# junhuihe2000/FLGP

Hardware: AMD Instinct MI355X
Metric: points/sec through k-NN->Laplacian->trunc-SVD->heat-cov, n=1e6 d=16 K=200 (higher is better)
Workload: dtype f64

## Files before the change

flgp_amd/_lib.py:

```python
from __future__ import annotations

import ctypes
import os

_HERE = os.path.dirname(os.path.abspath(__file__))
LIB_PATH = os.path.join(_HERE, "libflgp_hip.so")

c_int, c_double, c_long, c_void_p, c_char_p, c_size_t = (
    ctypes.c_int, ctypes.c_double, ctypes.c_long, ctypes.c_void_p, ctypes.c_char_p, ctypes.c_size_t)

P = c_void_p
_SIGNATURES = {
    "flgp_last_error": (c_char_p, []),
    "flgp_version": (c_char_p, []),
    "flgp_device_count": (c_int, []),
    "flgp_dev_pool_release": (c_size_t, []),
    "flgp_release_pinned": (None, []),
    "flgp_set_device": (c_int, [c_int]),
    "flgp_parse_gl": (c_int, [c_char_p]),
    "flgp_set_tuning": (c_int, [c_char_p, c_int]),
    "flgp_prof_enable": (None, [c_int]),
    "flgp_prof_reset": (None, []),
    "flgp_prof_query": (c_int, [c_char_p, P, P, P]),
    "flgp_prof_names": (c_int, [P, c_int]),
# ... 115 lines not shown
    "flgp_dev_gram_pack": (c_int, [P, P, P, c_int, c_int, P]),
    "flgp_dev_sym_pack": (c_int, [P, P, c_int, c_int, P]),
    "flgp_dev_sym_unpack": (c_int, [P, P, c_int, P, c_int]),
    "flgp_dev_eig_workspace": (c_size_t, [c_int, c_int]),
    "flgp_dev_eig_topk": (c_int, [P, P, c_int, c_int, c_int, c_double, P, P, c_int, P, c_size_t, P]),
    "flgp_dev_eig_plan": (c_int, [c_int, c_int, P]),
    "flgp_dev_bsg_workspace": (c_size_t, [c_int, c_int]),
    "flgp_dev_bsg_set_trace": (None, [P]),
    "flgp_dev_jac_set_trace": (None, [P]),
    "flgp_dev_bsg_apply": (c_int, [P, P, c_int, c_int, P, c_int, c_double, c_double, P, P, P, c_size_t, P]),
    "flgp_dev_u_recover_workspace": (c_size_t, [c_int, c_int]),
    "flgp_dev_u_recover_route": (c_int, [c_int, c_int, c_int, c_int, c_int]),
    "flgp_dev_spectrum_usable": (c_int, [P, P, c_int]),
    "flgp_dev_spectrum_usable_route": (c_int, [P, P, c_int, c_int]),
    "flgp_dev_u_recover": (c_int, [P, P, P, c_int, c_int, P, c_int, c_int, P, c_int, c_double, c_int, P, c_int, P, P]),
    "flgp_dev_hk": (c_int, [P, P, c_int, c_double, P, c_int, P, c_int, c_int, P, c_int, P, c_int, c_int,
                            P, c_int, P]),
    "flgp_dev_cholesky": (c_int, [P, P, c_int, c_int, P]),
    "flgp_dev_chol_solve": (c_int, [P, P, c_int, P, c_int, c_int, P]),
    "flgp_dev_tri_inverse_workspace": (c_size_t, [c_int]),
    "flgp_dev_tri_inverse": (c_int, [P, P, c_int, P, P, c_size_t, P]),
    "flgp_dev_gemm": (c_int, [P, c_int, c_int, c_int, c_double, P, c_long, c_long, P, c_long, c_long,
                              c_double, P, c_long, c_long, P, c_long, c_long, P, c_size_t]),
    "flgp_dev_rotate": (c_int, [P, c_int, c_int, c_double, P, P, P, c_double, P, P, P]),
    "flgp_dev_gram_small": (c_int, [P, c_int, c_int, P, P, P, P, c_size_t]),
    "flgp_dev_gemm_pair": (c_int, [P, c_int, c_int, c_int, c_double, P, P, c_long, c_long, P, P, c_long, c_long, P, P, c_long, c_long]),
    "flgp_dev_gemm_ex": (c_int, [P, c_int, c_int, c_int, c_double, P, c_long, c_long, P, c_long, c_long,
                                 c_double, P, c_long, c_long, P, c_long, c_long, P, c_size_t, c_double,
                                 P, c_int, c_int, P, P, P, P, P, P, P, ctypes.POINTER(c_int)]),
    "flgp_dev_gram_small_fused": (c_int, [P, c_int, c_int, P, P, P, P, c_size_t, c_int, P, P, P, P]),
# ... 61 lines not shown
```

flgp_amd/csrc/capi.hip:

```cpp
#include "common.h"
#include <chrono>
#include <memory>
#include <cstring>
#include <cmath>
#include <string>
#include <thread>
#include <vector>

using namespace flgp;

extern "C" int flgp_dev_spectrum_usable_route(void *stream, const double *d_eig, int K, int full_decomposition) {
  hipStream_t st = (hipStream_t)stream;
  FLGP_REQUIRE(d_eig && K >= 1, "spectrum_usable: bad arguments");
  std::vector<double> hv((size_t)K);
  FLGP_HIP(hipMemcpyAsync(hv.data(), d_eig, sizeof(double) * (size_t)K, hipMemcpyDeviceToHost, st));
  FLGP_HIP(hipStreamSynchronize(st));
  const double top = hv[0], low = hv[K - 1];
  if (!(top > 0.0) || !std::isfinite(top)) { set_error("spectrum: the similarity matrix is zero or not finite"); return FLGP_ERR_INVALID; }
  const double floor_rel = full_decomposition ? std::pow(10.0, -(double)tuning("spectrum_floor_exp_full", 13))
                                              : std::pow(10.0, -(double)tuning("spectrum_floor_exp", 10));
  if (!(low > floor_rel * top)) {
    set_error("spectrum: sigma_%d^2 = %.3e is below %.0e sigma_1^2 (= %.3e), what the %s resolves: K = %d reaches into the "
              "(numerical) null space of the similarity matrix, whose left vectors the Gram route cannot recover -- choose a "
              "smaller K", K, low, floor_rel, top, full_decomposition ? "full decomposition" : "block eigensolver", K);
// ... 206 lines not shown
  return laplacian(S, st, gl, sizes);
}

int csr_out(Sim &S, hipStream_t st, int *csr_p, int *csr_j, double *csr_x) {
  FLGP_TRY(d2h(csr_j, S.ell_idx.p, sizeof(int) * (size_t)S.n * S.r, st));
  FLGP_TRY(d2h(csr_x, S.ell_val.p, sizeof(double) * (size_t)S.n * S.r, st));
  FLGP_HIP(hipStreamSynchronize(st));
  if (csr_p)
    for (long i = 0; i <= S.n; ++i) csr_p[i] = (int)(i * S.r);
  return FLGP_OK;
}

struct Spectrum {
  DevBuf G, rec, eig, V, values, vectors, work, uwork;
  int K = 0;
};

int spectrum(Sim &S, hipStream_t st, int K, int root, Spectrum &P, int *info) {
  if (K < 0) K = S.s;
  FLGP_REQUIRE(K >= 1 && K <= S.s, "need 1 <= K <= s (K=%d, s=%d)", K, S.s);
  P.K = K;
  FLGP_TRY(build_csc_async(S, st));
  FLGP_TRY(colsum_of(S, st, S.ell_idx.as<int>(), S.ell_val.as<double>()));
  FLGP_TRY(flgp_comm_all_reduce_sum(S.comm, S.colsum.as<double>(), (size_t)S.s, st));
  FLGP_TRY(keep_colsum(S, st, S.keep_colsum_spectrum));
  FLGP_TRY(flgp_dev_col_scale(st, S.ell_idx.as<int>(), S.ell_val.as<double>(), S.n, S.r, S.colsum.as<double>(), nullptr, 1));
  FLGP_TRY(P.G.alloc(sizeof(double) * (size_t)S.s * S.s));
  FLGP_TRY(join_csc(S, st));
  if (flgp_dev_gram_uses_records(S.s, S.r)) {
    FLGP_TRY(P.rec.alloc(flgp_dev_gram_record_bytes(S.n, S.r)));
    FLGP_TRY(flgp_dev_gram_pack(st, S.ell_idx.as<int>(), S.ell_val.as<double>(), S.n, S.r, P.rec.as<double>()));
  }
  FLGP_TRY(flgp_dev_gram_ordered(st, S.ell_idx.as<int>(), S.ell_val.as<double>(), S.n, S.s, S.r, S.colptr.as<int>(),
// ... 5 lines not shown
    FLGP_TRY(flgp_dev_sym_pack(st, P.G.as<double>(), S.s, S.s, packed.as<double>()));
    FLGP_TRY(flgp_comm_all_reduce_sum(S.comm, packed.as<double>(), cnt, st));
    FLGP_TRY(flgp_dev_sym_unpack(st, packed.as<double>(), S.s, P.G.as<double>(), S.s));
    FLGP_HIP(hipStreamSynchronize(st));
  }
  const size_t wb = flgp_dev_eig_workspace(S.s, K);
  FLGP_TRY(P.work.alloc(wb));
  FLGP_TRY(P.eig.alloc(sizeof(double) * (size_t)K));
  FLGP_TRY(P.V.alloc(sizeof(double) * (size_t)S.s * K));
  int solve_info[4] = {0, 0, 0, 0};
  FLGP_TRY(flgp_dev_eig_topk(st, P.G.as<double>(), S.s, S.s, K, 0.0, P.eig.as<double>(), P.V.as<double>(), S.s,
                             P.work.p, wb, solve_info));
  if (info) for (int q = 0; q < 4; ++q) info[q] = solve_info[q];
  FLGP_TRY(flgp_dev_spectrum_usable_route(st, P.eig.as<double>(), K, solve_info[2]));
  if (!P.values.p) FLGP_TRY(P.values.alloc(sizeof(double) * (size_t)K));
  if (!P.vectors.p) FLGP_TRY(P.vectors.alloc(sizeof(double) * (size_t)S.n * K));
  FLGP_TRY(P.uwork.alloc(flgp_dev_u_recover_workspace(S.s, K)));
  return flgp_dev_u_recover(st, S.ell_idx.as<int>(), S.ell_val.as<double>(), S.n, S.r, P.V.as<double>(), S.s, S.s,
                            P.eig.as<double>(), K, std::sqrt((double)(S.n_global ? S.n_global : (long)S.n)), root,
                            P.vectors.as<double>(), S.n, P.values.as<double>(), P.uwork.as<double>());
}

int parse_kernel(const char *kernel, int *se) {
  if (kernel && !strcmp(kernel, "lae")) { *se = 0; return FLGP_OK; }
  if (kernel && !strcmp(kernel, "se")) { *se = 1; return FLGP_OK; }
  set_error("The kernel type is not supported!");
  return FLGP_ERR_UNSUPPORTED;
}

double now_s() { return std::chrono::duration<double>(std::chrono::steady_clock::now().time_since_epoch()).count(); }

struct HostSpectrum {
  Stream st;
  Sim S;
  Spectrum P;
// ... 632 lines not shown
  if (glc < 0) return glc;
  FLGP_REQUIRE(dX_loc && dU && dH_loc, "sharded covariance: null pointer");
  FLGP_REQUIRE(n_loc >= 1 && ldx >= n_loc && d >= 1 && s >= 1 && ldu >= s, "sharded covariance: bad shape n_loc=%d d=%d s=%d", n_loc, d, s);
  FLGP_REQUIRE(n_global >= n_loc && row_lo >= 0 && row_lo + n_loc <= n_global, "sharded covariance: rows [%ld, %ld) do not lie in [0, %ld)",
               row_lo, row_lo + n_loc, n_global);
  FLGP_REQUIRE(m >= 1 && (long)m <= n_global && ldh >= n_loc, "sharded covariance: need 1 <= m <= n and ldh >= n_loc");
  FLGP_REQUIRE(glc != FLGP_GL_CLUSTER_NORMALIZED || d_sizes, "gl=\"cluster-normalized\" needs the cluster sizes");
  FLGP_REQUIRE(!d_vectors_out || ldv >= n_loc, "sharded covariance: ldv < n_loc");
  if (K < 0) K = s;
  Sim S;
  S.n = n_loc; S.d = d; S.s = s; S.ldx = ldx; S.comm = comm; S.n_global = n_global; S.sizes = d_sizes;
  S.X.borrow(dX_loc);
  FLGP_TRY(anchor_panel(st, dU, s, ldu, d, S.Ut, S.uu));
  S.want_csc = true;
  FLGP_TRY(cross_similarity(S, st, r, se, glc, epsilon, d));
  Spectrum P;
  FLGP_TRY(spectrum(S, st, K, root, P, info));
  DevBuf V1, work;
  FLGP_TRY(V1.alloc(sizeof(double) * (size_t)m * K));
  FLGP_HIP(hipMemsetAsync(V1.p, 0, sizeof(double) * (size_t)m * K, st));
  if (row_lo < m) {
    const long cnt = std::min<long>(row_lo + n_loc, (long)m) - row_lo;
    FLGP_HIP(hipMemcpy2DAsync(V1.as<double>() + row_lo, sizeof(double) * (size_t)m, P.vectors.p, sizeof(double) * (size_t)n_loc,
                              sizeof(double) * (size_t)cnt, K, hipMemcpyDeviceToDevice, st));
  }
  FLGP_TRY(flgp_comm_all_reduce_sum(comm, V1.as<double>(), (size_t)m * K, st));
  FLGP_TRY(work.alloc(flgp_dev_hk_workspace(n_loc, m, K, 0)));
  FLGP_TRY(flgp_dev_hk(st, P.values.as<double>(), K, t, P.vectors.as<double>(), n_loc, nullptr, 0, n_loc, V1.as<double>(), m, nullptr, 0,
                       m, dH_loc, ldh, work.as<double>()));
  if (d_values_out) FLGP_HIP(hipMemcpyAsync(d_values_out, P.values.p, sizeof(double) * (size_t)K, hipMemcpyDeviceToDevice, st));
  if (d_vectors_out)
    FLGP_HIP(hipMemcpy2DAsync(d_vectors_out, sizeof(double) * (size_t)ldv, P.vectors.p, sizeof(double) * (size_t)n_loc,
                              sizeof(double) * (size_t)n_loc, K, hipMemcpyDeviceToDevice, st));
  FLGP_HIP(hipStreamSynchronize(st));
  return FLGP_OK;
}

extern "C" int flgp_heat_kernel_covariance_rank(const flgp_comm *comm, const double *X_rows, long ldx_host, int n_loc,
                                                long n_global, long row_lo, int m, int d, const double *U, int s, int ucols,
                                                int r, double t, int K, const char *kernel, const char *gl, int root,
                                                double epsilon, double *H_rows, long ldh_host, int *info) {
  const int world = comm ? comm->world : 1;
  Stream st;
  DevBuf dX, dUall, dHl;
// ... 212 lines not shown
```

flgp_amd/csrc/common.h:

```cpp
#pragma once
#include <hip/hip_runtime.h>
#include <cstdarg>
#include <cstdio>
#include <cstring>
#include <vector>
#include "../../include/flgp_hip.h"
#include "worker_pool.h"

namespace flgp {

void set_error(const char *fmt, ...);
int tuning(const char *key, int dflt);

struct DeviceFigures { int cus, lds_per_block; };
DeviceFigures device_figures();

int prof_begin(const char *name, hipStream_t st, double work);
void prof_end(int idx, hipStream_t st);
struct ProfScope {
  int idx; hipStream_t st;
  ProfScope(const char *name, hipStream_t s, double work) : idx(prof_begin(name, s, work)), st(s) {}
  ~ProfScope() { prof_end(idx, st); }
};

// ... 153 lines not shown
                 GemmFusedReduce *fused);
bool rot_applicable(int s, int b, const double *X, const double *X2, const double *WT, const double *out, const double *out2);
int rot_launch(hipStream_t st, int s, int b, double alpha, const double *X, const double *X2, const double *WT, double beta,
               const double *E, const double *E2, double *out, double *out2);
constexpr int GEMM_DIST_PARTS = 32;
struct GemmFusedReduce {
  int mode;
  double *dinv, *dist, *scratch;
  int *counter;
  bool done;
};

bool hk_panel_applicable(int n0, int n1, int K, long ldh);
bool hk_panel2_applicable(int n0, int n1, int K, long ldh);
size_t hk_panel_vw_elems(int n1, int K);
int hk_panel2_launch(hipStream_t st, const double *d_values, int K, double t, const double *V0, long ld0, int n0,
                     const double *dV1, int ld1, const int *d_idx1, int row0_1, int n1, double *dH, long ldh,
                     double *d_vw);
int hk_panel_launch(hipStream_t st, const double *d_values, int K, double t, const double *V0, long ld0, int n0,
                    const double *dV1, int ld1, const int *d_idx1, int row0_1, int n1, double *dH, long ldh,
                    double *d_vw);

int hk_ranges_to_host(hipStream_t st, const double *d_values, int K, double t, const double *d_vectors, int ldv,
                      int row0_0, int n0, int row0_1, int n1, double *H);
int d2h_cols_pipelined(hipStream_t st, const double *dM, long rows, int cols, double *H, long ldh, int rings_at_least);

int chol_solve(hipStream_t st, double *dA, int N, double *dB, int nrhs, int *d_flag);
int gpr_weights(hipStream_t st, const double *d_values, int K, double t, double *d_ls, double *d_l);
int gpr_q(hipStream_t st, const double *dVtV, const double *d_ls, int K, double c, double *dQ);
int gpr_scale(hipStream_t st, const double *dM, const double *d_a, const double *d_b, int rows, int cols, double *d_out);
// ... 174 lines not shown
```

flgp_amd/csrc/gemm.hip:

```cpp
#include "common.h"
#include <type_traits>

namespace flgp {

typedef double d4 __attribute__((ext_vector_type(4)));
typedef double d2 __attribute__((ext_vector_type(2)));

constexpr int GB = 128;
constexpr int GK = 16;
#ifndef GEMM_GLD_PAD
#define GEMM_GLD_PAD 17
#endif
constexpr int gld_of(int gbt) { return gbt + GEMM_GLD_PAD; }

struct GemmArgs {
  int M, N, Kd;
  const double *A; long a_is, a_ks;
  const double *B; long b_ks, b_js;
  double alpha, beta, gamma;
  const double *E; long e_is, e_js;
  const double *E2;
  double *C; long c_is, c_js;
  int shift_edges;
  int ksplit_len;
// ... 583 lines not shown
    FLGP_TRY(check_launch("splitk_reduce_kernel"));
  }
  return FLGP_OK;
}

__global__ void hk_scale_kernel(const double *__restrict__ values, int K, double t, const double *__restrict__ V1,
                                int ld1, const int *__restrict__ idx1, int row0, int n1, double *__restrict__ Vw) {
  const long e = (long)blockIdx.x * blockDim.x + threadIdx.x;
  if (e >= (long)n1 * K) return;
  const int b = (int)(e % n1), k = (int)(e / n1);
  const int row = idx1 ? idx1[b] : row0 + b;
  const double w = exp(-t * (1.0 - values[k]));
  Vw[e] = V1[(size_t)k * ld1 + row] * w;
}

__global__ void gather_rows_kernel(const double *__restrict__ V, int ld, const int *__restrict__ idx, int n0, int K,
                                   double *__restrict__ out, int ldo) {
  const long e = (long)blockIdx.x * blockDim.x + threadIdx.x;
  if (e >= (long)n0 * K) return;
  const int a = (int)(e % n0), k = (int)(e / n0);
  out[(size_t)k * ldo + a] = V[(size_t)k * ld + idx[a]];
}

}

using namespace flgp;

extern "C" int flgp_dev_gemm(void *stream, int M, int N, int Kd, double alpha, const double *A, long a_is,
                             long a_ks, const double *B, long b_ks, long b_js, double beta, const double *E,
                             long e_is, long e_js, double *C, long c_is, long c_js, double *d_work,
// ... 85 lines not shown
  double *Vw = d_work;
  const double *V0 = dV0 + row0_0;
  long v0_ld = ld0;
  if (d_idx0) {
    double *G0 = d_work + hk_panel_vw_elems(n1, K);
    hipLaunchKernelGGL(gather_rows_kernel, dim3(ceil_div((long)n0 * K, 256)), dim3(256), 0, st, dV0, ld0, d_idx0,
                       n0, K, G0, n0);
    FLGP_TRY(check_launch("gather_rows_kernel"));
    V0 = G0;
    v0_ld = n0;
  }
  if (hk_panel2_applicable(n0, n1, K, ldh))
    return hk_panel2_launch(st, d_values, K, t, V0, v0_ld, n0, dV1, ld1, d_idx1, row0_1, n1, dH, ldh, Vw);
  if (hk_panel_applicable(n0, n1, K, ldh))
    return hk_panel_launch(st, d_values, K, t, V0, v0_ld, n0, dV1, ld1, d_idx1, row0_1, n1, dH, ldh, Vw);
  hipLaunchKernelGGL(hk_scale_kernel, dim3(ceil_div((long)n1 * K, 256)), dim3(256), 0, st, d_values, K, t, dV1, ld1,
                     d_idx1, row0_1, n1, Vw);
  FLGP_TRY(check_launch("hk_scale_kernel"));
  return gemm_launch(st, n0, n1, K, 1.0, V0, 1, v0_ld, Vw, n1, 1, 0.0, nullptr, 0, 0, dH, 1, ldh, nullptr, 0, 0.0,
                     nullptr);
}
```

flgp_amd/csrc/sparse.hip:

```cpp
#include "common.h"

namespace flgp {

__global__ __launch_bounds__(256) void csc_hist_kernel(const int *__restrict__ ell_idx, long nnz, int s,
                                                       int chunk, int *__restrict__ hist) {
  extern __shared__ int lh[];
  for (int j = threadIdx.x; j < s; j += blockDim.x) lh[j] = 0;
  __syncthreads();
  const long e0 = (long)blockIdx.x * chunk;
  long e1 = e0 + chunk;
  if (e1 > nnz) e1 = nnz;
  for (long e = e0 + threadIdx.x; e < e1; e += blockDim.x) atomicAdd(&lh[ell_idx[e]], 1);
  __syncthreads();
  int *out = hist + (size_t)blockIdx.x * s;
  for (int j = threadIdx.x; j < s; j += blockDim.x) out[j] = lh[j];
}

__global__ void csc_colscan_kernel(int *__restrict__ hist, int nchunks, int s, int *__restrict__ tot) {
  const int j = blockIdx.x * blockDim.x + threadIdx.x;
  if (j >= s) return;
  int run = 0;
  constexpr int CB = 16;
  int c = 0;
  for (; c + CB <= nchunks; c += CB) {
// ... 480 lines not shown
  }
  __syncthreads();
  for (int e = tid; e < KT * ROWS; e += 256) {
    const int kq = e / ROWS, i = e % ROWS;
    if (k0 + kq < K && i0 + i < n) out[(size_t)(k0 + kq) * ldo + i0 + i] = tile[kq][i];
  }
}

#ifndef U_RECOVER_LDS_THREADS
#define U_RECOVER_LDS_THREADS 1024
#endif
#ifndef U_RECOVER_LDS_MIN_N
#define U_RECOVER_LDS_MIN_N 10000
#endif
constexpr int U_LDS_BYTES = 163840;

static int u_lds_width(int s) {
  const long w = s >= 1 ? (long)U_LDS_BYTES / (8L * s) : 0;
  return w > 4 ? 4 : (int)w;
}

template <int W>
__global__ __launch_bounds__(256) void transpose_v_slices_kernel(const double *__restrict__ V, int ldv, int s, int K,
                                                                 double *__restrict__ Vts) {
  const int j = blockIdx.x * 256 + threadIdx.x, sl = blockIdx.y;
  if (j >= s) return;
  double *o = Vts + ((size_t)sl * s + j) * W;
#pragma unroll
  for (int c = 0; c < W; ++c) {
    const int k = sl * W + c;
    o[c] = k < K ? V[(size_t)k * ldv + j] : 0.0;
  }
}

template <int W> __device__ __forceinline__ int u_lds_slot(int q) { return W == 4 ? q ^ (((q >> 5) & 1) << 1) : q; }

template <int W, int NP>
__global__ __launch_bounds__(U_RECOVER_LDS_THREADS) void u_recover_lds_kernel(const int *__restrict__ ell_idx,
                                                                              const double *__restrict__ val, int n, int r, int s,
                                                                              const double *__restrict__ Vts,
                                                                              const double *__restrict__ eig, int K, double scale,
                                                                              double *__restrict__ out, int ldo, int rows_per_range) {
  typedef double d2u __attribute__((ext_vector_type(2), aligned(8)));
  typedef int i2u __attribute__((ext_vector_type(2), aligned(4)));
  typedef double d2 __attribute__((ext_vector_type(2)));
  extern __shared__ __attribute__((aligned(16))) double u_slice[];
  const int tid = threadIdx.x, T = blockDim.x, sl = blockIdx.y;
  const double *src = Vts + (size_t)sl * s * W;
  for (int q = tid; q < s * W; q += T) u_slice[u_lds_slot<W>(q)] = src[q];
  double sg[W];
#pragma unroll
  for (int c = 0; c < W; ++c) {
    const int k = sl * W + c;
    const double e = k < K ? eig[k] : 0.0;
    sg[c] = __builtin_sqrt(e > 0.0 ? e : 0.0);
  }
  __syncthreads();
  const long i_lo = (long)blockIdx.x * rows_per_range;
  const long i_hi = (i_lo + rows_per_range < n) ? i_lo + rows_per_range : n;
  const long last_pair = (long)n * r - 2;
  constexpr int CE = 2 * NP;
  constexpr int GB = NP <= 4 ? CE : (W == 4 && NP == 6) ? 4 : NP;
  struct Chunk { double z0[NP], z1[NP]; int j0[NP], j1[NP]; };
  auto fetch = [&](long i, int ch) {
    Chunk c;
#pragma unroll
    for (int u = 0; u < NP; ++u) {
      const int a = CE * ch + 2 * u;
      long b = (i < i_hi && a < r) ? i * r + a : i_lo * r;
// ... 46 lines not shown
#pragma unroll
        for (int h = 0; h < 2; ++h)
          if (2 * u + h < left) {
            double z, v[W];
            gather(cur, u, h, moved, z, v);
#pragma unroll
            for (int c = 0; c < W; ++c) acc[c] += z * v[c];
          }
      }
    }
    if (ch == nch - 1) {
      if (i < i_hi) {
#pragma unroll
        for (int c = 0; c < W; ++c) {
          const int k = sl * W + c;
          if (k < K) out[(size_t)k * ldo + i] = sg[c] > 0.0 ? (acc[c] / sg[c]) * scale : 0.0;
        }
      }
#pragma unroll
      for (int c = 0; c < W; ++c) acc[c] = 0.0;
    }
  };
  const long nit = i_hi > i_lo ? (i_hi - i_lo + T - 1) / T : 0;
  const long steps = nit * nch;
  long ia = i_lo + tid; int cha = 0;
  auto next = [&](long &i, int &ch) { if (++ch == nch) { ch = 0; i += T; } };
  Chunk A = fetch(ia, cha), B;
  for (long t = 0; t < steps; t += 2) {
    long ib = ia; int chb = cha; next(ib, chb);
    B = fetch(ib, chb);
    apply(A, ia, cha);
    ia = ib; cha = chb; next(ia, cha);
    A = fetch(ia, cha);
    if (t + 1 < steps) apply(B, ib, chb);
  }
}

__global__ void values_out_kernel(const double *__restrict__ eig, int K, int root, double *__restrict__ values) {
  const int k = blockIdx.x * blockDim.x + threadIdx.x;
  if (k >= K) return;
  const double ev = eig[k] > 0.0 ? eig[k] : 0.0;
  values[k] = root ? __builtin_sqrt(ev) : ev;
}

struct CscPlan {
  int nchunks, chunk, nbits;
  size_t hist_bytes, tot_bytes;
};

static CscPlan csc_plan(long nnz, int s) {
  CscPlan p;
  long nc = (nnz + 2047) / 2048;
  if (nc > 2048) nc = 2048;
  if (nc < 1) nc = 1;
  long chunk = (nnz + nc - 1) / nc;
  chunk = (chunk + 63) / 64 * 64;
  if (chunk < 64) chunk = 64;
// ... 238 lines not shown
  int dev = 0;
  if (hipGetDevice(&dev) != hipSuccess || dev < 0 || dev >= 16) return 256;
  if (!cus[dev]) {
    int c = 0;
    cus[dev] = (hipDeviceGetAttribute(&c, hipDeviceAttributeMultiprocessorCount, dev) == hipSuccess && c > 0) ? c : 256;
  }
  return cus[dev];
}

constexpr int U_LDS_MAX_PAIRS = 6;
static int u_lds_pairs(int r) {
  const int pairs = (r + 1) / 2, steps = ceil_div(pairs, U_LDS_MAX_PAIRS);
  return ceil_div(pairs, steps);
}

template <int W, int NP>
static int u_recover_lds_launch(hipStream_t st, const int *d_ell_idx, const double *d_ell_val, int n, int r, const double *dV,
                                int ldv, int s, const double *d_eig, int K, double scale, double *d_vectors, int ldo,
                                double *d_work) {
  const int slices = ceil_div(K, W);
  hipLaunchKernelGGL((transpose_v_slices_kernel<W>), dim3(ceil_div(s, 256), slices), dim3(256), 0, st, dV, ldv, s, K, d_work);
  FLGP_TRY(check_launch("transpose_v_slices_kernel"));
  int ranges = num_cus() / slices;
  if (ranges < 1) ranges = 1;
  int rows = ceil_div(ceil_div(n, ranges), 64) * 64;
  ranges = ceil_div(n, rows);
  const size_t lds = sizeof(double) * (size_t)s * W;
  if (lds > 48 * 1024)
    FLGP_HIP(hipFuncSetAttribute((const void *)u_recover_lds_kernel<W, NP>, hipFuncAttributeMaxDynamicSharedMemorySize, (int)lds));
  hipLaunchKernelGGL((u_recover_lds_kernel<W, NP>), dim3(ranges, slices), dim3(U_RECOVER_LDS_THREADS), lds, st, d_ell_idx, d_ell_val,
                     n, r, s, d_work, d_eig, K, scale, d_vectors, ldo, rows);
  return FLGP_OK;
}

template <int W>
static int u_recover_lds_pairs(hipStream_t st, const int *d_ell_idx, const double *d_ell_val, int n, int r, const double *dV,
                               int ldv, int s, const double *d_eig, int K, double scale, double *d_vectors, int ldo,
                               double *d_work) {
  switch (u_lds_pairs(r)) {
#define U_LDS_PAIRS(NPv)                                                                                                       \
  case NPv: return u_recover_lds_launch<W, NPv>(st, d_ell_idx, d_ell_val, n, r, dV, ldv, s, d_eig, K, scale, d_vectors, ldo, d_work)
    U_LDS_PAIRS(1); U_LDS_PAIRS(2); U_LDS_PAIRS(3); U_LDS_PAIRS(4); U_LDS_PAIRS(5);
    default: U_LDS_PAIRS(6);
#undef U_LDS_PAIRS
  }
}

extern "C" int flgp_dev_u_recover(void *stream, const int *d_ell_idx, const double *d_ell_val, int n, int r,
                                  const double *dV, int ldv, int s, const double *d_eig, int K, double scale,
                                  int root, double *d_vectors, int ldo, double *d_values_out, double *d_work) {
  hipStream_t st = (hipStream_t)stream;
  FLGP_REQUIRE(r >= 1 && r <= FLGP_RMAX && K >= 1 && ldo >= n, "u_recover: bad shape");
  if (n > 0) {
    ProfScope ps("u_recover_kernel", st, 12.0 * (double)n * r + 8.0 * (double)s * K + 8.0 * (double)n * K);
    const int route = flgp_dev_u_recover_route(n, r, s, K, d_work != nullptr);
    if (route == 4) {
      switch (u_lds_width(s)) {
#define U_LDS_CASE(Wv)                                                                                                         \
  case Wv: FLGP_TRY(u_recover_lds_pairs<Wv>(st, d_ell_idx, d_ell_val, n, r, dV, ldv, s, d_eig, K, scale, d_vectors, ldo, d_work)); break
        U_LDS_CASE(1); U_LDS_CASE(2); U_LDS_CASE(3);
        default: U_LDS_CASE(4);
#undef U_LDS_CASE
      }
    } else if (d_work) {
      hipLaunchKernelGGL(transpose_v_kernel, dim3(ceil_div(s, 32), ceil_div(K, 32)), dim3(256), 0, st, dV, ldv, s, K,
                         d_work);
      if (K % 4 == 0) {
        hipLaunchKernelGGL((u_recover_wide_kernel<4, 32>), dim3(ceil_div(n, 32), ceil_div(K, 256)), dim3(256), 0, st, d_ell_idx,
                           d_ell_val, n, r, d_work, d_eig, K, scale, d_vectors, ldo);
      } else if (K % 2 == 0) {
        hipLaunchKernelGGL((u_recover_wide_kernel<2, 64>), dim3(ceil_div(n, 64), ceil_div(K, 128)), dim3(256), 0, st, d_ell_idx,
                           d_ell_val, n, r, d_work, d_eig, K, scale, d_vectors, ldo);
      } else {
        hipLaunchKernelGGL(u_recover_tiled_kernel, dim3(ceil_div(n, 64), ceil_div(K, 64)), dim3(256), 0, st, d_ell_idx,
                           d_ell_val, n, r, d_work, d_eig, K, scale, d_vectors, ldo);
      }
    } else {
      hipLaunchKernelGGL(u_recover_kernel, dim3(ceil_div(n, 256), ceil_div(K, 8)), dim3(256), 0, st, d_ell_idx,
                         d_ell_val, n, r, dV, ldv, d_eig, K, scale, d_vectors, ldo);
    }
    FLGP_TRY(check_launch("u_recover_kernel"));
  }
  if (d_values_out) {
    hipLaunchKernelGGL(values_out_kernel, dim3(ceil_div(K, 256)), dim3(256), 0, st, d_eig, K, root, d_values_out);
    FLGP_TRY(check_launch("values_out_kernel"));
  }
  return FLGP_OK;
}
```

flgp_amd/pipeline.py:

```python
from __future__ import annotations

import math
import time
from dataclasses import dataclass, field

import torch

from . import _lib

GL_CODES = {"rw": 0, "normalized": 1, "cluster-normalized": 2}


def shard_bounds(n: int, world: int, rank: int):
    base, rem = divmod(n, world)
    lo = rank * base + min(rank, rem)
    return lo, lo + base + (1 if rank < rem else 0)


class HipStages:

    def __init__(self, device):
        self.device = torch.device(device)
        if self.device.type != "cuda":
            raise RuntimeError("HipStages needs a GPU: the HIP library is the only implementation of this path")
# ... 118 lines not shown
        work = self.empty((self.L.flgp_dev_u_recover_workspace(s, K) // 8 + 1,))
        _lib.check(self.L.flgp_dev_spectrum_usable_route(self._st(), eig.data_ptr(), K, int(bool(dense))))
        _lib.check(self.L.flgp_dev_u_recover(self._st(), ell_idx.data_ptr(), ell_val.data_ptr(), n, r, V.data_ptr(), s, s,
                                             eig.data_ptr(), K, float(scale), int(bool(root)), vectors.data_ptr(), max(n, 1),
                                             values.data_ptr(), work.data_ptr()))
        return values, vectors

    def hk(self, values, t, V0, V1):
        K, n0 = V0.shape
        n1 = V1.shape[1]
        H = self.empty((n1, n0))
        wb = self.L.flgp_dev_hk_workspace(n0, n1, K, 0)
        work = self.empty((wb // 8 + 1,))
        _lib.check(self.L.flgp_dev_hk(self._st(), values.data_ptr(), K, float(t), V0.data_ptr(), n0, None, 0, n0,
                                      V1.data_ptr(), n1, None, 0, n1, H.data_ptr(), n0, work.data_ptr()))
        return H

    def nystrom(self, X, U, a2, K):
        d, n = X.shape
        s = U.shape[1]
        values = self.empty((K,)); vectors = self.empty((K, max(n, 1)))
        if n:
            _lib.check(self.L.flgp_dev_nystrom_eigenpair(self._st(), X.data_ptr(), n, n, d, U.data_ptr(), s, s, float(a2), int(K),
                                                         values.data_ptr(), vectors.data_ptr(), n))
        return values, vectors

    def nystrom_grid(self, U, a2s, K, max_parallel=10, owner=None):
        import ctypes
        import numpy as np
        self.nystrom_grid_free(owner)
# ... 211 lines not shown
        if self.dist and self.world > 1:
            G = S.sym_unpack(self._all_reduce(S.sym_pack(G)), G)
        tm.mark("gram")
        K = s if cfg.K < 0 else cfg.K
        eig, V, info = S.eig_topk(G, K)
        tm.mark("eig")
        values, vectors = S.u_recover(ell_idx, ell_val, V, eig, math.sqrt(float(n_global)), cfg.root, dense=info.get("dense"))
        tm.mark("u_recover")
        m = cfg.m
        V1 = torch.zeros((K, m), dtype=vectors.dtype, device=vectors.device)
        lo, hi = row_lo, row_lo + n_loc
        if lo < m:
            cnt = min(hi, m) - lo
            V1[:, lo:lo + cnt] = vectors[:, :cnt]
        self._all_reduce(V1)
        H = S.hk(values, cfg.t, vectors[:, :n_loc].contiguous() if vectors.shape[1] != n_loc else vectors, V1)
        tm.mark("heat_kernel")
        res = PathResult(values=values, vectors=vectors, H=H, stage_ms=tm.result(), eig_info=info)
        if keep:
            res.ell_idx, res.ell_val, res.knn_idx, res.G = ell_idx, ell_val, knn_idx, G
        return res


class NystromPath(HeatKernelPath):

    def run_nystrom(self, X_loc, U, a2: float, K: int):
        return self.stages.nystrom(X_loc, U, a2, K)

    def run_nystrom_grid(self, X_train_loc, U, a2s, K: int, max_parallel: int = 10):
        values, mean = self.stages.nystrom_grid(U, a2s, K, max_parallel, owner=self)
        return values, self.stages.nystrom_grid_extend_all(X_train_loc, owner=self), mean
# ... 13 lines not shown
```

include/flgp_hip.h:

```cpp
#ifndef FLGP_HIP_H
#define FLGP_HIP_H

#include <stddef.h>

#ifdef __cplusplus
extern "C" {
#endif

#define FLGP_OK 0
#define FLGP_ERR_INVALID (-1)
#define FLGP_ERR_NOMEM (-2)
#define FLGP_ERR_UNSUPPORTED (-3)
#define FLGP_ERR_HIP (-4)
#define FLGP_ERR_NOCONV (-5)
#define FLGP_ERR_PEER (-6)

#define FLGP_RMAX 32
#define FLGP_SMAX 32768
#define FLGP_DMAX 16384

#define FLGP_GL_RW 0
#define FLGP_GL_NORMALIZED 1
#define FLGP_GL_CLUSTER_NORMALIZED 2

// ... 255 lines not shown

size_t flgp_dev_bsg_workspace(int s, int b);
void flgp_dev_bsg_set_trace(void *d_trace);
void flgp_dev_jac_set_trace(void *d_trace);
int flgp_dev_bsg_apply(void *stream, const double *dG, int ldg, int s, const double *dX, int b, double alpha,
                       double beta, const double *dE, double *dOut, void *d_work, size_t work_bytes, int *info);

size_t flgp_dev_u_recover_workspace(int s, int K);
int flgp_dev_u_recover_route(int n, int r, int s, int K, int has_work);
int flgp_dev_spectrum_usable_route(void *stream, const double *d_eig, int K, int full_decomposition);
int flgp_dev_spectrum_usable(void *stream, const double *d_eig, int K);
int flgp_dev_u_recover(void *stream, const int *d_ell_idx, const double *d_ell_val, int n, int r,
                       const double *dV, int ldv, int s, const double *d_eig, int K, double scale,
                       int root, double *d_vectors, int ldo, double *d_values_out, double *d_work);

int flgp_dev_gather_rows(void *stream, const double *dV, int ld, const int *d_idx, int n0, int K, double *d_out);
size_t flgp_dev_hk_workspace(int n0, int n1, int K, int gather0);
int flgp_dev_cholesky(void *stream, double *d_A, int m, int single_workgroup, int *d_flag);
int flgp_dev_chol_solve(void *stream, const double *d_L, int m, double *d_B, int nrhs, int mode, const int *d_flag);
size_t flgp_dev_tri_inverse_workspace(int m);
int flgp_dev_tri_inverse(void *stream, const double *d_L, int m, double *d_X, void *d_work, size_t work_bytes, const int *d_flag);
int flgp_dev_hk(void *stream, const double *d_values, int K, double t,
                const double *dV0, int ld0, const int *d_idx0, int row0_0, int n0,
                const double *dV1, int ld1, const int *d_idx1, int row0_1, int n1,
                double *dH, int ldh, double *d_work);

int flgp_dev_gemm(void *stream, int M, int N, int Kd, double alpha,
                  const double *A, long a_is, long a_ks, const double *B, long b_ks, long b_js,
                  double beta, const double *E, long e_is, long e_js, double *C, long c_is, long c_js,
                  double *d_work, size_t work_elems);
// ... 59 lines not shown
```

Before: 40.28 million.

## Compute heat kernel rows via sparse product with precomputed s-by-m panel

Adds an hk_rows path that reassociates the heat-covariance product. It first forms B = V·diag(scale/sigma) (s×K), then Wm = B·(V1 scaled by the heat weights) (s×m), and finally applies the sparse ELL similarity rows to Wm with the existing LDS u-recover kernel in a raw mode. This avoids materialising the full n×K eigenvector matrix and running the n×m×K dense GEMM, and it limits u_recover to the rows the anchor block needs. A tuning-based route heuristic decides when the path is used, and it adds workspace and template variants.

```diff
diff --git a/flgp_amd/_lib.py b/flgp_amd/_lib.py
--- a/flgp_amd/_lib.py
+++ b/flgp_amd/_lib.py
@@ -153,6 +153,10 @@
     "flgp_dev_spectrum_usable": (c_int, [P, P, c_int]),
     "flgp_dev_spectrum_usable_route": (c_int, [P, P, c_int, c_int]),
     "flgp_dev_u_recover": (c_int, [P, P, P, c_int, c_int, P, c_int, c_int, P, c_int, c_double, c_int, P, c_int, P, P]),
+    "flgp_dev_hk_rows_workspace": (c_size_t, [c_int, c_int, c_int]),
+    "flgp_dev_hk_rows_route": (c_int, [c_int, c_int, c_int, c_int, c_int]),
+    "flgp_dev_hk_rows": (c_int, [P, P, P, c_int, c_int, P, c_int, c_int, P, c_int, c_double, P, c_double, P, c_int, c_int,
+                                 P, c_int, P]),
     "flgp_dev_hk": (c_int, [P, P, c_int, c_double, P, c_int, P, c_int, c_int, P, c_int, P, c_int, c_int,
                             P, c_int, P]),
     "flgp_dev_cholesky": (c_int, [P, P, c_int, c_int, P]),
diff --git a/flgp_amd/csrc/capi.hip b/flgp_amd/csrc/capi.hip
--- a/flgp_amd/csrc/capi.hip
+++ b/flgp_amd/csrc/capi.hip
@@ -244,9 +244,10 @@
 struct Spectrum {
   DevBuf G, rec, eig, V, values, vectors, work, uwork;
   int K = 0;
+  int vec_rows = 0;
 };
 
-int spectrum(Sim &S, hipStream_t st, int K, int root, Spectrum &P, int *info) {
+int spectrum(Sim &S, hipStream_t st, int K, int root, Spectrum &P, int *info, int row_limit = -1) {
   if (K < 0) K = S.s;
   FLGP_REQUIRE(K >= 1 && K <= S.s, "need 1 <= K <= s (K=%d, s=%d)", K, S.s);
   P.K = K;
@@ -282,11 +283,12 @@
   if (info) for (int q = 0; q < 4; ++q) info[q] = solve_info[q];
   FLGP_TRY(flgp_dev_spectrum_usable_route(st, P.eig.as<double>(), K, solve_info[2]));
   if (!P.values.p) FLGP_TRY(P.values.alloc(sizeof(double) * (size_t)K));
-  if (!P.vectors.p) FLGP_TRY(P.vectors.alloc(sizeof(double) * (size_t)S.n * K));
+  P.vec_rows = row_limit >= 0 && row_limit < S.n ? row_limit : S.n;
+  if (!P.vectors.p) FLGP_TRY(P.vectors.alloc(sizeof(double) * (size_t)std::max(P.vec_rows, 1) * K));
   FLGP_TRY(P.uwork.alloc(flgp_dev_u_recover_workspace(S.s, K)));
-  return flgp_dev_u_recover(st, S.ell_idx.as<int>(), S.ell_val.as<double>(), S.n, S.r, P.V.as<double>(), S.s, S.s,
+  return flgp_dev_u_recover(st, S.ell_idx.as<int>(), S.ell_val.as<double>(), P.vec_rows, S.r, P.V.as<double>(), S.s, S.s,
                             P.eig.as<double>(), K, std::sqrt((double)(S.n_global ? S.n_global : (long)S.n)), root,
-                            P.vectors.as<double>(), S.n, P.values.as<double>(), P.uwork.as<double>());
+                            P.vectors.as<double>(), std::max(P.vec_rows, 1), P.values.as<double>(), P.uwork.as<double>());
 }
 
 int parse_kernel(const char *kernel, int *se) {
@@ -949,20 +951,27 @@
   FLGP_TRY(anchor_panel(st, dU, s, ldu, d, S.Ut, S.uu));
   S.want_csc = true;
   FLGP_TRY(cross_similarity(S, st, r, se, glc, epsilon, d));
+  const int hk_rows = flgp_dev_hk_rows_route(n_loc, r, s, K, m);
+  const long own = row_lo < m ? std::min<long>(row_lo + n_loc, (long)m) - row_lo : 0;
   Spectrum P;
-  FLGP_TRY(spectrum(S, st, K, root, P, info));
+  FLGP_TRY(spectrum(S, st, K, root, P, info, hk_rows && !d_vectors_out ? (int)own : -1));
   DevBuf V1, work;
   FLGP_TRY(V1.alloc(sizeof(double) * (size_t)m * K));
   FLGP_HIP(hipMemsetAsync(V1.p, 0, sizeof(double) * (size_t)m * K, st));
-  if (row_lo < m) {
-    const long cnt = std::min<long>(row_lo + n_loc, (long)m) - row_lo;
-    FLGP_HIP(hipMemcpy2DAsync(V1.as<double>() + row_lo, sizeof(double) * (size_t)m, P.vectors.p, sizeof(double) * (size_t)n_loc,
-                              sizeof(double) * (size_t)cnt, K, hipMemcpyDeviceToDevice, st));
-  }
+  if (own > 0)
+    FLGP_HIP(hipMemcpy2DAsync(V1.as<double>() + row_lo, sizeof(double) * (size_t)m, P.vectors.p, sizeof(double) * (size_t)P.vec_rows,
+                              sizeof(double) * (size_t)own, K, hipMemcpyDeviceToDevice, st));
   FLGP_TRY(flgp_comm_all_reduce_sum(comm, V1.as<double>(), (size_t)m * K, st));
-  FLGP_TRY(work.alloc(flgp_dev_hk_workspace(n_loc, m, K, 0)));
-  FLGP_TRY(flgp_dev_hk(st, P.values.as<double>(), K, t, P.vectors.as<double>(), n_loc, nullptr, 0, n_loc, V1.as<double>(), m, nullptr, 0,
-                       m, dH_loc, ldh, work.as<double>()));
+  if (hk_rows) {
+    FLGP_TRY(work.alloc(flgp_dev_hk_rows_workspace(s, m, K)));
+    FLGP_TRY(flgp_dev_hk_rows(st, S.ell_idx.as<int>(), S.ell_val.as<double>(), n_loc, S.r, P.V.as<double>(), s, s, P.eig.as<double>(), K,
+                              std::sqrt((double)n_global), P.values.as<double>(), t, V1.as<double>(), m, m, dH_loc, ldh,
+                              work.as<double>()));
+  } else {
+    FLGP_TRY(work.alloc(flgp_dev_hk_workspace(n_loc, m, K, 0)));
+    FLGP_TRY(flgp_dev_hk(st, P.values.as<double>(), K, t, P.vectors.as<double>(), n_loc, nullptr, 0, n_loc, V1.as<double>(), m, nullptr,
+                         0, m, dH_loc, ldh, work.as<double>()));
+  }
   if (d_values_out) FLGP_HIP(hipMemcpyAsync(d_values_out, P.values.p, sizeof(double) * (size_t)K, hipMemcpyDeviceToDevice, st));
   if (d_vectors_out)
     FLGP_HIP(hipMemcpy2DAsync(d_vectors_out, sizeof(double) * (size_t)ldv, P.vectors.p, sizeof(double) * (size_t)n_loc,
diff --git a/flgp_amd/csrc/common.h b/flgp_amd/csrc/common.h
--- a/flgp_amd/csrc/common.h
+++ b/flgp_amd/csrc/common.h
@@ -191,6 +191,8 @@
 bool hk_panel_applicable(int n0, int n1, int K, long ldh);
 bool hk_panel2_applicable(int n0, int n1, int K, long ldh);
 size_t hk_panel_vw_elems(int n1, int K);
+int hk_scale_launch(hipStream_t st, const double *d_values, int K, double t, const double *dV1, int ld1, const int *d_idx1,
+                    int row0_1, int n1, double *d_vw);
 int hk_panel2_launch(hipStream_t st, const double *d_values, int K, double t, const double *V0, long ld0, int n0,
                      const double *dV1, int ld1, const int *d_idx1, int row0_1, int n1, double *dH, long ldh,
                      double *d_vw);
diff --git a/flgp_amd/csrc/gemm.hip b/flgp_amd/csrc/gemm.hip
--- a/flgp_amd/csrc/gemm.hip
+++ b/flgp_amd/csrc/gemm.hip
@@ -621,6 +621,13 @@
   Vw[e] = V1[(size_t)k * ld1 + row] * w;
 }
 
+int hk_scale_launch(hipStream_t st, const double *d_values, int K, double t, const double *dV1, int ld1, const int *d_idx1,
+                    int row0_1, int n1, double *d_vw) {
+  hipLaunchKernelGGL(hk_scale_kernel, dim3(ceil_div((long)n1 * K, 256)), dim3(256), 0, st, d_values, K, t, dV1, ld1,
+                     d_idx1, row0_1, n1, d_vw);
+  return check_launch("hk_scale_kernel");
+}
+
 __global__ void gather_rows_kernel(const double *__restrict__ V, int ld, const int *__restrict__ idx, int n0, int K,
                                    double *__restrict__ out, int ldo) {
   const long e = (long)blockIdx.x * blockDim.x + threadIdx.x;
@@ -736,9 +743,7 @@
     return hk_panel2_launch(st, d_values, K, t, V0, v0_ld, n0, dV1, ld1, d_idx1, row0_1, n1, dH, ldh, Vw);
   if (hk_panel_applicable(n0, n1, K, ldh))
     return hk_panel_launch(st, d_values, K, t, V0, v0_ld, n0, dV1, ld1, d_idx1, row0_1, n1, dH, ldh, Vw);
-  hipLaunchKernelGGL(hk_scale_kernel, dim3(ceil_div((long)n1 * K, 256)), dim3(256), 0, st, d_values, K, t, dV1, ld1,
-                     d_idx1, row0_1, n1, Vw);
-  FLGP_TRY(check_launch("hk_scale_kernel"));
+  FLGP_TRY(hk_scale_launch(st, d_values, K, t, dV1, ld1, d_idx1, row0_1, n1, Vw));
   return gemm_launch(st, n0, n1, K, 1.0, V0, 1, v0_ld, Vw, n1, 1, 0.0, nullptr, 0, 0, dH, 1, ldh, nullptr, 0, 0.0,
                      nullptr);
 }
diff --git a/flgp_amd/csrc/sparse.hip b/flgp_amd/csrc/sparse.hip
--- a/flgp_amd/csrc/sparse.hip
+++ b/flgp_amd/csrc/sparse.hip
@@ -518,6 +518,7 @@
 #define U_RECOVER_LDS_MIN_N 10000
 #endif
 constexpr int U_LDS_BYTES = 163840;
+constexpr int HK_ROWS_MIN_KW_PER_R = 60, HK_ROWS_MIN_KW_PER_R_SMALL_M = 40, HK_ROWS_PANEL2_M = 480, HK_ROWS_MIN_M = 100;
 
 static int u_lds_width(int s) {
   const long w = s >= 1 ? (long)U_LDS_BYTES / (8L * s) : 0;
@@ -539,7 +540,7 @@
 
 template <int W> __device__ __forceinline__ int u_lds_slot(int q) { return W == 4 ? q ^ (((q >> 5) & 1) << 1) : q; }
 
-template <int W, int NP>
+template <int W, int NP, bool RAW>
 __global__ __launch_bounds__(U_RECOVER_LDS_THREADS) void u_recover_lds_kernel(const int *__restrict__ ell_idx,
                                                                               const double *__restrict__ val, int n, int r, int s,
                                                                               const double *__restrict__ Vts,
@@ -556,7 +557,7 @@
 #pragma unroll
   for (int c = 0; c < W; ++c) {
     const int k = sl * W + c;
-    const double e = k < K ? eig[k] : 0.0;
+    const double e = (!RAW && k < K) ? eig[k] : 0.0;
     sg[c] = __builtin_sqrt(e > 0.0 ? e : 0.0);
   }
   __syncthreads();
@@ -633,7 +634,7 @@
 #pragma unroll
         for (int c = 0; c < W; ++c) {
           const int k = sl * W + c;
-          if (k < K) out[(size_t)k * ldo + i] = sg[c] > 0.0 ? (acc[c] / sg[c]) * scale : 0.0;
+          if (k < K) out[(size_t)k * ldo + i] = RAW ? acc[c] : sg[c] > 0.0 ? (acc[c] / sg[c]) * scale : 0.0;
         }
       }
 #pragma unroll
@@ -660,6 +661,17 @@
   if (k >= K) return;
   const double ev = eig[k] > 0.0 ? eig[k] : 0.0;
   values[k] = root ? __builtin_sqrt(ev) : ev;
+}
+
+__global__ void hk_rows_b_kernel(const double *__restrict__ Vs, int ldv, int s, const double *__restrict__ eig, int K,
+                                 double scale, double *__restrict__ B) {
+  const long e = (long)blockIdx.x * blockDim.x + threadIdx.x;
+  if (e >= (long)s * K) return;
+  const int j = (int)(e % s), k = (int)(e / s);
+  const double ev = eig[k];
+  const double sigma = __builtin_sqrt(ev > 0.0 ? ev : 0.0);
+  const double q = sigma > 0.0 ? scale / sigma : 0.0;
+  B[e] = Vs[(size_t)k * ldv + j] * q;
 }
 
 struct CscPlan {
@@ -928,7 +940,7 @@
   return ceil_div(pairs, steps);
 }
 
-template <int W, int NP>
+template <int W, int NP, bool RAW>
 static int u_recover_lds_launch(hipStream_t st, const int *d_ell_idx, const double *d_ell_val, int n, int r, const double *dV,
                                 int ldv, int s, const double *d_eig, int K, double scale, double *d_vectors, int ldo,
                                 double *d_work) {
@@ -941,22 +953,35 @@
   ranges = ceil_div(n, rows);
   const size_t lds = sizeof(double) * (size_t)s * W;
   if (lds > 48 * 1024)
-    FLGP_HIP(hipFuncSetAttribute((const void *)u_recover_lds_kernel<W, NP>, hipFuncAttributeMaxDynamicSharedMemorySize, (int)lds));
-  hipLaunchKernelGGL((u_recover_lds_kernel<W, NP>), dim3(ranges, slices), dim3(U_RECOVER_LDS_THREADS), lds, st, d_ell_idx, d_ell_val,
+    FLGP_HIP(hipFuncSetAttribute((const void *)u_recover_lds_kernel<W, NP, RAW>, hipFuncAttributeMaxDynamicSharedMemorySize, (int)lds));
+  hipLaunchKernelGGL((u_recover_lds_kernel<W, NP, RAW>), dim3(ranges, slices), dim3(U_RECOVER_LDS_THREADS), lds, st, d_ell_idx, d_ell_val,
                      n, r, s, d_work, d_eig, K, scale, d_vectors, ldo, rows);
   return FLGP_OK;
 }
 
-template <int W>
+template <int W, bool RAW>
 static int u_recover_lds_pairs(hipStream_t st, const int *d_ell_idx, const double *d_ell_val, int n, int r, const double *dV,
                                int ldv, int s, const double *d_eig, int K, double scale, double *d_vectors, int ldo,
                                double *d_work) {
   switch (u_lds_pairs(r)) {
 #define U_LDS_PAIRS(NPv)                                                                                                       \
-  case NPv: return u_recover_lds_launch<W, NPv>(st, d_ell_idx, d_ell_val, n, r, dV, ldv, s, d_eig, K, scale, d_vectors, ldo, d_work)
+  case NPv: return u_recover_lds_launch<W, NPv, RAW>(st, d_ell_idx, d_ell_val, n, r, dV, ldv, s, d_eig, K, scale, d_vectors, ldo, d_work)
     U_LDS_PAIRS(1); U_LDS_PAIRS(2); U_LDS_PAIRS(3); U_LDS_PAIRS(4); U_LDS_PAIRS(5);
     default: U_LDS_PAIRS(6);
 #undef U_LDS_PAIRS
+  }
+}
+
+template <bool RAW>
+static int u_recover_lds_width(hipStream_t st, const int *d_ell_idx, const double *d_ell_val, int n, int r, const double *dV,
+                               int ldv, int s, const double *d_eig, int K, double scale, double *d_vectors, int ldo,
+                               double *d_work) {
+  switch (u_lds_width(s)) {
+#define U_LDS_CASE(Wv)                                                                                                         \
+  case Wv: return u_recover_lds_pairs<Wv, RAW>(st, d_ell_idx, d_ell_val, n, r, dV, ldv, s, d_eig, K, scale, d_vectors, ldo, d_work)
+    U_LDS_CASE(1); U_LDS_CASE(2); U_LDS_CASE(3);
+    default: U_LDS_CASE(4);
+#undef U_LDS_CASE
   }
 }
 
@@ -969,13 +994,7 @@
     ProfScope ps("u_recover_kernel", st, 12.0 * (double)n * r + 8.0 * (double)s * K + 8.0 * (double)n * K);
     const int route = flgp_dev_u_recover_route(n, r, s, K, d_work != nullptr);
     if (route == 4) {
-      switch (u_lds_width(s)) {
-#define U_LDS_CASE(Wv)                                                                                                         \
-  case Wv: FLGP_TRY(u_recover_lds_pairs<Wv>(st, d_ell_idx, d_ell_val, n, r, dV, ldv, s, d_eig, K, scale, d_vectors, ldo, d_work)); break
-        U_LDS_CASE(1); U_LDS_CASE(2); U_LDS_CASE(3);
-        default: U_LDS_CASE(4);
-#undef U_LDS_CASE
-      }
+      FLGP_TRY(u_recover_lds_width<false>(st, d_ell_idx, d_ell_val, n, r, dV, ldv, s, d_eig, K, scale, d_vectors, ldo, d_work));
     } else if (d_work) {
       hipLaunchKernelGGL(transpose_v_kernel, dim3(ceil_div(s, 32), ceil_div(K, 32)), dim3(256), 0, st, dV, ldv, s, K,
                          d_work);
@@ -1001,3 +1020,48 @@
   }
   return FLGP_OK;
 }
+
+namespace {
+struct HkRowsLayout { size_t b, vw, wm, image, total; };
+HkRowsLayout hk_rows_layout(int s, int m, int K) {
+  auto up = [](size_t e) { return (e + 31) / 32 * 32; };
+  const int w = u_lds_width(s);
+  const size_t S = s > 0 ? s : 0, M = m > 0 ? m : 0, Kk = K > 0 ? K : 0;
+  HkRowsLayout L;
+  L.b = 0;
+  L.vw = L.b + up(S * Kk);
+  L.wm = L.vw + up(M * Kk);
+  L.image = L.wm + up(S * M);
+  L.total = L.image + up(S * (w >= 1 ? (size_t)ceil_div(M, w) * w : M));
+  return L;
+}
+}
+
+extern "C" size_t flgp_dev_hk_rows_workspace(int s, int m, int K) { return sizeof(double) * hk_rows_layout(s, m, K).total + 256; }
+
+extern "C" int flgp_dev_hk_rows_route(int n, int r, int s, int K, int m) {
+  const int knob = tuning("hk_rows", 1);
+  const int w = u_lds_width(s);
+  if (!knob || w < 1 || n < U_RECOVER_LDS_MIN_N || (long)n * r < 2 || r < 1 || r > FLGP_RMAX || K < 1 || m < 1) return 0;
+  if (knob == 2) return 1;
+  if (m < HK_ROWS_MIN_M) return 0;
+  return (long)K * w >= (m >= HK_ROWS_PANEL2_M ? HK_ROWS_MIN_KW_PER_R : HK_ROWS_MIN_KW_PER_R_SMALL_M) * (long)r;
+}
+
+extern "C" int flgp_dev_hk_rows(void *stream, const int *d_ell_idx, const double *d_ell_val, int n, int r, const double *dVs,
+                                int ldv, int s, const double *d_eig, int K, double scale, const double *d_values, double t,
+                                const double *dV1, int ld1, int m, double *dH, int ldh, double *d_work) {
+  hipStream_t st = (hipStream_t)stream;
+  FLGP_REQUIRE(d_ell_idx && d_ell_val && dVs && d_eig && d_values && dV1 && dH && d_work, "hk_rows: null pointer");
+  FLGP_REQUIRE(r >= 1 && r <= FLGP_RMAX && K >= 1 && m >= 1 && s >= 1 && ldv >= s && ld1 >= m && ldh >= n, "hk_rows: bad shape");
+  FLGP_REQUIRE(u_lds_width(s) >= 1 && n >= U_RECOVER_LDS_MIN_N && (long)n * r >= 2,
+               "hk_rows: no LDS slice for n=%d r=%d s=%d (ask flgp_dev_hk_rows_route)", n, r, s);
+  const HkRowsLayout L = hk_rows_layout(s, m, K);
+  double *B = d_work + L.b, *Vw = d_work + L.vw, *Wm = d_work + L.wm, *image = d_work + L.image;
+  hipLaunchKernelGGL(hk_rows_b_kernel, dim3(ceil_div((long)s * K, 256)), dim3(256), 0, st, dVs, ldv, s, d_eig, K, scale, B);
+  FLGP_TRY(check_launch("hk_rows_b_kernel"));
+  FLGP_TRY(hk_scale_launch(st, d_values, K, t, dV1, ld1, nullptr, 0, m, Vw));
+  FLGP_TRY(gemm_launch(st, s, m, K, 1.0, B, 1, s, Vw, m, 1, 0.0, nullptr, 0, 0, Wm, 1, s, nullptr, 0, 0.0, nullptr));
+  ProfScope ps("hk_rows_kernel", st, 2.0 * (double)n * r * m);
+  return u_recover_lds_width<true>(st, d_ell_idx, d_ell_val, n, r, Wm, s, s, nullptr, m, 1.0, dH, ldh, image);
+}
diff --git a/flgp_amd/pipeline.py b/flgp_amd/pipeline.py
--- a/flgp_amd/pipeline.py
+++ b/flgp_amd/pipeline.py
@@ -156,6 +156,20 @@
         work = self.empty((wb // 8 + 1,))
         _lib.check(self.L.flgp_dev_hk(self._st(), values.data_ptr(), K, float(t), V0.data_ptr(), n0, None, 0, n0,
                                       V1.data_ptr(), n1, None, 0, n1, H.data_ptr(), n0, work.data_ptr()))
+        return H
+
+    def hk_rows_route(self, n, r, s, K, m):
+        return bool(self.L.flgp_dev_hk_rows_route(n, r, s, K, m))
+
+    def hk_rows(self, ell_idx, ell_val, V, eig, scale, values, t, V1):
+        n, r = ell_idx.shape
+        K, s = V.shape
+        m = V1.shape[1]
+        H = self.empty((m, n))
+        work = self.empty((self.L.flgp_dev_hk_rows_workspace(s, m, K) // 8 + 1,))
+        _lib.check(self.L.flgp_dev_hk_rows(self._st(), ell_idx.data_ptr(), ell_val.data_ptr(), n, r, V.data_ptr(), s, s, eig.data_ptr(),
+                                           K, float(scale), values.data_ptr(), float(t), V1.data_ptr(), m, m, H.data_ptr(), n,
+                                           work.data_ptr()))
         return H
 
     def nystrom(self, X, U, a2, K):
@@ -397,7 +411,10 @@
             cnt = min(hi, m) - lo
             V1[:, lo:lo + cnt] = vectors[:, :cnt]
         self._all_reduce(V1)
-        H = S.hk(values, cfg.t, vectors[:, :n_loc].contiguous() if vectors.shape[1] != n_loc else vectors, V1)
+        if hasattr(S, "hk_rows") and n_loc and S.hk_rows_route(n_loc, cfg.r, s, K, m):
+            H = S.hk_rows(ell_idx, ell_val, V, eig, math.sqrt(float(n_global)), values, cfg.t, V1)
+        else:
+            H = S.hk(values, cfg.t, vectors[:, :n_loc].contiguous() if vectors.shape[1] != n_loc else vectors, V1)
         tm.mark("heat_kernel")
         res = PathResult(values=values, vectors=vectors, H=H, stage_ms=tm.result(), eig_info=info)
         if keep:
diff --git a/include/flgp_hip.h b/include/flgp_hip.h
--- a/include/flgp_hip.h
+++ b/include/flgp_hip.h
@@ -293,6 +293,12 @@
                        const double *dV, int ldv, int s, const double *d_eig, int K, double scale,
                        int root, double *d_vectors, int ldo, double *d_values_out, double *d_work);
 
+size_t flgp_dev_hk_rows_workspace(int s, int m, int K);
+int flgp_dev_hk_rows_route(int n, int r, int s, int K, int m);
+int flgp_dev_hk_rows(void *stream, const int *d_ell_idx, const double *d_ell_val, int n, int r, const double *dVs, int ldv,
+                     int s, const double *d_eig, int K, double scale, const double *d_values, double t, const double *dV1,
+                     int ld1, int m, double *dH, int ldh, double *d_work);
+
 int flgp_dev_gather_rows(void *stream, const double *dV, int ld, const int *d_idx, int n0, int K, double *d_out);
 size_t flgp_dev_hk_workspace(int n0, int n1, int K, int gather0);
 int flgp_dev_cholesky(void *stream, double *d_A, int m, int single_workgroup, int *d_flag);
```

Result: faster. 44.99 million, median of 6 (+11.7%).
